# jeremy-rifkin/Markov-Huffman-Coding

Measured on AMD Instinct MI355X. Metric: encode+decode GB/s on 16 GB byte stream, bit-exact round-trip, higher is better.
Workload: dtype u8

## Files before the change

### markov-huffman-coding_amd/csrc/mh_index.hip

```cpp
#include "mh_decode_dev.hpp"

namespace mhk {

__device__ __forceinline__ uint64_t st_pack(uint32_t prev, uint64_t pos) { return (uint64_t(prev) << 56) | pos; }
__device__ __forceinline__ uint32_t st_shift(const IdxParams &p) { return p.order == 2 ? 48u : 56u; }
__device__ __forceinline__ uint64_t st_make(const IdxParams &p, uint32_t ctx, uint64_t pos) { return (uint64_t(ctx) << st_shift(p)) | pos; }
__device__ __forceinline__ uint64_t st_pos(const IdxParams &p, uint64_t s) { return s & ((1ull << st_shift(p)) - 1ull); }
__device__ __forceinline__ uint32_t st_ctx(const IdxParams &p, uint64_t s) { return uint32_t(s >> st_shift(p)); }

__device__ __forceinline__ void idx_fine_entry(const IdxParams &p, uint64_t g, uint32_t prev, uint64_t pos) {
    if (p.fine && p.order != 2 && (g & ((1u << T_SUB_SHIFT) - 1u)) == 0 && (g >> T_SUB_SHIFT) < p.fine_cap)
        p.fine[g >> T_SUB_SHIFT] = (prev << 24) | (uint32_t(pos) & FINE_POS_MASK);
}

template <typename F>
__device__ __forceinline__ uint64_t walk_segment(const IdxParams &p, const DecTables &tabs, const BitSrc &src, uint64_t start,
                                                 uint64_t seg_end, uint32_t &count, bool &bad, F on_symbol, uint32_t *max_used = nullptr) {
    uint64_t pos = st_pos(p, start);
    uint32_t prev = st_ctx(p, start);
    count = 0;
    bad = false;
    if (max_used) *max_used = 0;
    if (pos >= seg_end) return start;
    GranuleCursor bc;
// ... 356 lines not shown
    IdxWs w;
    w.nseg = (nbits + IDX_SEG_BITS_MIN - 1) / IDX_SEG_BITS_MIN;
    w.nblk = (w.nseg + SCAN_BLOCK - 1) / SCAN_BLOCK;
    auto up = [](size_t v) { return (v + 63) & ~size_t(63); };
    w.off_changed = 64;
    w.off_end = up(w.off_changed + IDX_MAX_PASSES * 4);
    w.off_used = up(w.off_end + size_t(w.nseg) * 8);
    w.off_count = up(w.off_used + size_t(w.nseg) * 8);
    w.off_start = up(w.off_count + size_t(w.nseg) * 4);
    w.off_blk = up(w.off_start + size_t(w.nseg) * 8);
    w.total = up(w.off_blk + size_t(w.nblk + 1) * 8);
    w.nseg5 = (nbits + IX_SEG_BITS - 1) / IX_SEG_BITS;
    w.ntile5 = (w.nseg5 + IX_TILE_SEGS - 1) / IX_TILE_SEGS;
    w.ntblk = (w.ntile5 + SCAN_BLOCK - 1) / SCAN_BLOCK;
    w.dirty_cap = w.nseg5 / 4 + 64;
    w.off_e16 = w.off_end;
    w.off_s16 = up(w.off_e16 + size_t(w.nseg5) * 2);
    w.off_c16 = up(w.off_s16 + size_t(w.nseg5) * 2);
    w.off_dirty = up(w.off_c16 + size_t(w.nseg5) * 2 + 64);
    w.off_dirty2 = up(w.off_dirty + size_t(w.dirty_cap) * 4);
    w.off_tcnt = up(w.off_dirty2 + size_t(w.dirty_cap) * 4);
    w.off_tbase = up(w.off_tcnt + size_t(w.ntile5) * 4);
    w.off_tblk = up(w.off_tbase + size_t(w.ntile5) * 8);
    const size_t total5 = up(w.off_tblk + size_t(w.ntblk + 1) * 8);
    if (total5 > w.total) w.total = total5;
    return w;
}
size_t build_index_workspace_bytes(uint64_t nbits) { return idx_ws_layout(nbits).total; }

static void note_index_path(unsigned char *ws, uint32_t path, hipStream_t st) {
    (void)launch_set_word(reinterpret_cast<uint32_t *>(ws + 8), path, st);
}

static bool index_tiles_eligible(const IdxParams &p, const IdxWs &L, uint32_t g, bool allow_long = false) {
    return p.order != 2 && p.tprim && p.tP == 7 && (allow_long || p.max_len <= p.tP + p.tH) && g == 1 && p.nbits >= (1ull << 20) && L.nseg5 < 0xFFFFFFFFull && !getenv("MH_INDEX_NO_TILES");
}
static hipError_t index_tile_states(const IdxParams &p, const IdxWs &L, unsigned char *ws, hipStream_t st, IdxParams &q, bool *ok_out) {
    hipError_t e = hipSuccess;
    q = p;
    q.e16 = reinterpret_cast<uint16_t *>(ws + L.off_e16);
    q.s16 = reinterpret_cast<uint16_t *>(ws + L.off_s16);
    q.c16 = reinterpret_cast<uint16_t *>(ws + L.off_c16);
    q.tile_cnt = reinterpret_cast<uint32_t *>(ws + L.off_tcnt);
    q.tile_base = reinterpret_cast<unsigned long long *>(ws + L.off_tbase);
    q.nseg5 = L.nseg5; q.ntile5 = L.ntile5;
    q.dirty_list = reinterpret_cast<uint32_t *>(ws + L.off_dirty);
    q.dirty_cap = uint32_t(L.dirty_cap < 0xFFFFFFFFull ? L.dirty_cap : 0xFFFFFFFFull);
    const uint64_t dwant = (q.nseg5 + 255) / 256;
    const unsigned dgrid = unsigned(dwant < 2048 ? dwant : 2048);
    bool ok = false;
    uint32_t it = 0;
    q.warm_bits = 256;
    if (const char *wv = getenv("MH_INDEX_WARM_BITS")) { const int v = atoi(wv); if (v >= 16 && v <= int(IX_WARM_BITS_MAX)) q.warm_bits = uint32_t(v); }
    else if (q.ntile5 >= 16384) {
        IdxParams sq = q;
        sq.ntile5 = q.ntile5 / 256 > 4096 ? q.ntile5 / 256 : 4096;
        sq.nseg5 = sq.ntile5 * IX_TILE_SEGS;
        sq.warm_bits = 96;
        sq.iter = it;
        e = launch_index_tile(sq, 0, st);
        if (e != hipSuccess) return e;
        hipLaunchKernelGGL(index_tile_dirty_kernel, dim3(256), dim3(256), 0, st, sq);
        unsigned int dirty = ~0u;
        e = hipMemcpyAsync(&dirty, q.changed + it, 4, hipMemcpyDeviceToHost, st);
        if (e == hipSuccess) e = hipStreamSynchronize(st);
        if (e != hipSuccess) return e;
        ++it;
        if (uint64_t(dirty) * 40u < sq.nseg5) q.warm_bits = 96;
// ... 279 lines not shown
```

### markov-huffman-coding_amd/csrc/mh_tile.hip

```cpp
#include <hip/hip_runtime.h>
#include <stdint.h>

#include <algorithm>
#include <cstdlib>
#include <mutex>
#include <utility>
#include <vector>

#include "mh_kernels.h"
#include "mh_model.hpp"

namespace mhk {

using mh::DEC16_LEAF;

constexpr int T_SUB = 1 << T_SUB_SHIFT;
constexpr int T_TILE = 64 * T_SUB;
constexpr int T_NU = T_SUB / 16;
constexpr int T_LPK = 1024 / T_SUB;
constexpr int T_NG = 64 / T_LPK;
static_assert(T_SUB == 32 || T_SUB == 64, "the output transposition below is written for 32- or 64-symbol sub-chunks");
constexpr int T_THREADS = 1024;
constexpr int T_WAVES = T_THREADS / 64;
constexpr int T_LDS_BYTES = 163840;
// ... 13 lines not shown
template <int O2>
__device__ __forceinline__ uint64_t sub_pos(const TileParams &p, uint64_t j, uint32_t f) {
    return sub_pos_of<O2>(p.index[(j << T_SUB_SHIFT) >> p.chunk_shift], f);
}

__device__ __forceinline__ uint64_t uniform64(uint64_t v) {
    const uint32_t lo = uint32_t(__builtin_amdgcn_readfirstlane(int(uint32_t(v))));
    const uint32_t hi = uint32_t(__builtin_amdgcn_readfirstlane(int(uint32_t(v >> 32))));
    return (uint64_t(hi) << 32) | lo;
}

__device__ __forceinline__ uint64_t stage_first(uint64_t start) { return (start >> 3) & ~uint64_t(15); }

typedef __attribute__((address_space(3))) const uint32_t lds_u32;
typedef uint32_t u32x4 __attribute__((ext_vector_type(4)));
template <typename T>
__device__ __forceinline__ __attribute__((address_space(3))) const T *lds_ptr(uint32_t byte_addr) {
    return reinterpret_cast<__attribute__((address_space(3))) const T *>(byte_addr);
}
template <typename T>
__device__ __forceinline__ __attribute__((address_space(3))) T *lds_wptr(uint32_t byte_addr) {
    return reinterpret_cast<__attribute__((address_space(3))) T *>(byte_addr);
}
__device__ __forceinline__ uint32_t lds_addr_of(const void *generic) {
    return uint32_t(reinterpret_cast<uintptr_t>((__attribute__((address_space(3))) const void *)(generic)));
}

__device__ __forceinline__ unsigned long long tile_stamp() {
    unsigned long long t;
    __builtin_amdgcn_sched_barrier(0);
    asm volatile("s_waitcnt vmcnt(0) lgkmcnt(0)\n\ts_memtime %0\n\ts_waitcnt lgkmcnt(0)" : "=s"(t) :: "memory");
    __builtin_amdgcn_sched_barrier(0);
    return t;
}

__device__ __forceinline__ uint32_t tile_put_byte(uint32_t d, uint32_t e, int j) {
    const uint32_t sel = j == 0 ? 0x03020104u : j == 1 ? 0x03020400u : j == 2 ? 0x03040100u : 0x04020100u;
    return __builtin_amdgcn_perm(e, d, sel);
}

#ifdef MH_EXP_PROBES
#include "mh_tile_probes.hpp"
#else
__host__ __device__ constexpr uint32_t tile_probe_reserve(int) { return 0u; }
#endif

template <int K, int PC, int HC, int OUT, int WIN, int STAMP = 0, int O2 = 0, int G = 0>
__global__ __launch_bounds__(T_THREADS) void decode_tile_kernel(TileParams p) {
    extern __shared__ __attribute__((aligned(16))) unsigned char smem[];
    constexpr uint32_t P = PC;
    const uint32_t PRIM_BYTES = O2 ? ((p.nslots << P) * 4u + 15u) & ~15u : (256u << P) * 2u;
    const uint32_t tid = threadIdx.x, lane = tid & 63u, wave = tid >> 6;
    if (p.d_nbits) {
        p.nbits = *p.d_nbits;
        p.payload_bytes = (p.nbits + 7) >> 3;
    }
    uint16_t *lut = reinterpret_cast<uint16_t *>(smem);
    for (uint32_t i = tid; i < PRIM_BYTES / 16u; i += T_THREADS)
        reinterpret_cast<uint4 *>(lut)[i] = reinterpret_cast<const uint4 *>(p.prim)[i];
    __syncthreads();
    const uint64_t nsub = (p.n + T_SUB - 1) >> T_SUB_SHIFT;
    constexpr uint32_t RESERVE = tile_probe_reserve(G);
    const uint32_t free_bytes = uint32_t(T_LDS_BYTES) - PRIM_BYTES - RESERVE;
    uint32_t maxb;
    {
        uint32_t *s_max = reinterpret_cast<uint32_t *>(smem + PRIM_BYTES + RESERVE);
// ... 321 lines not shown
                        const u32x4 v = *lds_ptr<u32x4>(rb + l * uint32_t(T_SUB) + ((u ^ swz(l)) << 4));
                        reinterpret_cast<uint4 *>(p.out + ((j0 + uint64_t(k) * 64u + uint32_t(g) * uint32_t(T_LPK)) << T_SUB_SHIFT))[lane] = make_uint4(v.x, v.y, v.z, v.w);
                        __builtin_amdgcn_wave_barrier();
                        asm volatile("" ::: "memory");
                    }
                }
            }
            if (STAMP) { const unsigned long long t4 = tile_stamp(); seg[2] += t3 - t2; seg[3] += t4 - t3; }
            land_ahead(seg[1], seg[0]);
        } else {
            if (mc.cls == 1u) {
                if (lane == 0) atomicExch(p.status, MHK_STATUS_CORRUPT);
            } else {
                const uint64_t c0 = (tc * TSYM) >> p.chunk_shift;
                for (uint32_t c = lane; c < chunks_per_tile * K; c += 64) p.redo[1u + atomicAdd(p.redo, 1u)] = uint32_t(c0 + c);
            }
            fetch_ahead();
            land_ahead(seg[1], seg[0]);
        }
    }
    if (STAMP && lane == 0) {
        unsigned long long *dst = reinterpret_cast<unsigned long long *>(p.status) + 1;
        for (int i = 0; i < 4; ++i) atomicAdd(&dst[i], seg[i]);
    }
}

constexpr uint32_t IX_TILE_BYTES = IX_TILE_BITS / 8;
constexpr uint32_t IX_STAGE_LEAD = IX_WARM_BITS_MAX / 8;
constexpr uint32_t IX_STAGE_BYTES = IX_TILE_BYTES + IX_STAGE_LEAD + 32u;
constexpr uint32_t IX_REGION = IX_STAGE_BYTES + 16u;
static_assert(IX_STAGE_LEAD % 16 == 0 && IX_STAGE_BYTES % 16 == 0 && IX_TILE_BYTES % 16 == 0, "16-byte staging loads");
static_assert(IX_TILE_SEGS == 128, "two segments per lane");

template <int MODE, int PC>
__global__ __launch_bounds__(T_THREADS) void index_tile_kernel(IdxParams p) {
    extern __shared__ __attribute__((aligned(16))) unsigned char smem[];
    constexpr uint32_t P = PC, PRIM_BYTES = (256u << P) * 2u;
    constexpr int K = 2;
    const uint32_t tid = threadIdx.x, lane = tid & 63u, wave = tid >> 6;
    for (uint32_t i = tid; i < PRIM_BYTES / 16u; i += T_THREADS)
        reinterpret_cast<uint4 *>(smem)[i] = reinterpret_cast<const uint4 *>(p.tprim)[i];
    __syncthreads();
    constexpr uint32_t NW = (uint32_t(T_LDS_BYTES) - PRIM_BYTES) / IX_REGION < uint32_t(T_WAVES) ? (uint32_t(T_LDS_BYTES) - PRIM_BYTES) / IX_REGION : uint32_t(T_WAVES);
    if (wave >= NW) return;
    if (lds_addr_of(smem) != 0u) {
        if (tid == 0) atomicExch(p.status, MHK_STATUS_CORRUPT);
        return;
    }
    unsigned char *reg = smem + PRIM_BYTES + wave * IX_REGION;
    const uint32_t reg_bit0 = lds_addr_of(reg) * 8u;
    const uint32_t H = p.tH;
    const __amdgpu_buffer_rsrc_t sec_rsrc =
        __builtin_amdgcn_make_buffer_rsrc(const_cast<uint16_t *>(p.tsec), 0, p.tnsec ? int((p.tnsec + 8u) * 2u) : 0, 0x00020000);
    const uint64_t vec_total = (p.payload_bytes + 15u) >> 4;
    const uint64_t cmask = (1ull << p.chunk_shift) - 1ull;

    for (uint64_t t = uint64_t(blockIdx.x) * NW + wave; t < p.ntile5; t += uint64_t(gridDim.x) * NW) {
        const uint64_t sb = t ? t * IX_TILE_BYTES - IX_STAGE_LEAD : 0ull;
        {
            const uint4 *src = reinterpret_cast<const uint4 *>(p.payload + sb);
            const uint64_t left = vec_total - (sb >> 4);
            const uint32_t nvec = left < IX_STAGE_BYTES / 16u ? uint32_t(left) : IX_STAGE_BYTES / 16u;
            for (uint32_t i = lane; i < IX_REGION / 16u; i += 64u) {
                uint4 v = make_uint4(0, 0, 0, 0);
                if (i < nvec) {
                    v = src[i];
                    v.x = __builtin_bswap32(__builtin_bitreverse32(v.x));
                    v.y = __builtin_bswap32(__builtin_bitreverse32(v.y));
                    v.z = __builtin_bswap32(__builtin_bitreverse32(v.z));
                    v.w = __builtin_bswap32(__builtin_bitreverse32(v.w));
                }
                *reinterpret_cast<uint4 *>(reg + i * 16u) = v;
            }
        }
        uint64_t seg[K], base[K];
        uint32_t qb0[K], qe0[K], q[K], ctx[K], k[K], S[K], badv[K], want_e[K], want_c[K], next_entry[K];
        bool active[K], last[K];
#pragma unroll
        for (int j = 0; j < K; ++j) {
            seg[j] = t * IX_TILE_SEGS + uint32_t(j) * 64u + lane;
            const uint64_t b0 = seg[j] * IX_SEG_BITS;
            active[j] = b0 < p.nbits;
            const uint64_t e0 = b0 + IX_SEG_BITS < p.nbits ? b0 + IX_SEG_BITS : p.nbits;
            last[j] = active[j] && e0 == p.nbits;
            qb0[j] = reg_bit0 + uint32_t(b0 - sb * 8u);
            qe0[j] = active[j] ? reg_bit0 + uint32_t(e0 - sb * 8u) : qb0[j];
            k[j] = 0; S[j] = IX_INVALID; badv[j] = DEC16_LEAF; base[j] = 0; want_e[j] = want_c[j] = next_entry[j] = 0;
            if (MODE == 0) {
                const bool exact = seg[j] == 0;
                ctx[j] = exact ? p.prev0 : 0x20u;
                const uint32_t room = qb0[j] - reg_bit0;
                q[j] = exact || !active[j] ? qb0[j] : qb0[j] - (p.warm_bits < room ? p.warm_bits : room);
            } else {
                uint32_t pe = p.prev0 << 8;
                if (active[j] && seg[j]) pe = p.e16[seg[j] - 1];
                ctx[j] = pe >> 8;
                q[j] = active[j] ? qb0[j] + (pe & 255u) : qb0[j];
                want_e[j] = active[j] ? p.e16[seg[j]] : 0u;
                want_c[j] = active[j] ? (p.c16[seg[j]] & IX_C16_COUNT) : 0u;
            }
        }
        if (MODE == 1) {
            uint64_t run = p.tile_base[t];
#pragma unroll
            for (int j = 0; j < K; ++j) {
                uint32_t inc = want_c[j];
#pragma unroll
                for (int d = 1; d < 64; d <<= 1) { const uint32_t o = __shfl_up(inc, d); if (lane >= uint32_t(d)) inc += o; }
                base[j] = run + (inc - want_c[j]);
                next_entry[j] = (0u - uint32_t(base[j])) & ((1u << T_SUB_SHIFT) - 1u);
                run += __shfl(inc, 63);
            }
        }
        uint32_t overflow = 0;
        auto step = [&](auto entered_c) __attribute__((always_inline)) {
            constexpr bool ENTERED = decltype(entered_c)::value;
            if (MODE == 1) {
#pragma unroll
                for (int j = 0; j < K; ++j) {
                    if (q[j] < qe0[j] && k[j] == next_entry[j]) {
                        next_entry[j] += 1u << T_SUB_SHIFT;
                        const uint64_t g = base[j] + k[j];
                        const uint64_t pos = sb * 8u + (q[j] - reg_bit0);
                        if ((g & cmask) == 0) {
                            const uint64_t ci = g >> p.chunk_shift;
                            if (ci < p.index_cap) p.index[ci] = (uint64_t(ctx[j]) << 56) | pos; else overflow = 1;
                        }
                        if (p.fine && (g >> T_SUB_SHIFT) < p.fine_cap) p.fine[g >> T_SUB_SHIFT] = (ctx[j] << 24) | (uint32_t(pos) & FINE_POS_MASK);
                    }
                }
            }
            uint32_t w0[K], w1[K], win[K], e[K], e2[K];
#pragma unroll
            for (int j = 0; j < K; ++j) {
                const lds_u32 *wp = lds_ptr<uint32_t>((q[j] >> 3) & ~3u);
                w0[j] = wp[0];
                w1[j] = wp[1];
            }
            __builtin_amdgcn_sched_barrier(0);
#pragma unroll
            for (int j = 0; j < K; ++j) {
                win[j] = __builtin_amdgcn_alignbit(w1[j], w0[j], q[j]);
                e[j] = *lds_ptr<uint16_t>(((win[j] << 1) & ((2u << P) - 2u)) | (ctx[j] << (P + 1)));
            }
            __builtin_amdgcn_sched_barrier(0);
#pragma unroll
            for (int j = 0; j < K; ++j) {
// ... 11 lines not shown
                    q[j] += __builtin_amdgcn_ubfe(efm, 8, 5);
                    ctx[j] = efm & 255u;
                    k[j] += go ? 1u : 0u;
                } else {
                    const bool in = q[j] >= qb0[j];
                    if (MODE == 0) S[j] = (in && S[j] == IX_INVALID) ? ((ctx[j] << 8) | (q[j] - qb0[j])) : S[j];
                    const uint32_t len = __builtin_amdgcn_ubfe(ef, 8, 5);
                    const bool ok = (ef & DEC16_LEAF) != 0u;
                    badv[j] &= (in && go && !ok) ? 0u : ~0u;
                    ctx[j] = (ok && go) ? (ef & 255u) : ctx[j];
                    q[j] += go ? (ok ? len : 1u) : 0u;
                    k[j] += (in && go) ? 1u : 0u;
                }
            }
        };
        uint32_t it = 0;
        if (MODE == 0) {
#pragma unroll 1
            for (; it < IX_WARM_BITS_MAX + 64u; it += 4u) {
                if (__all(q[0] >= qb0[0] && q[1] >= qb0[1])) break;
#pragma unroll
                for (int sub = 0; sub < 4; ++sub) step(std::false_type{});
            }
#pragma unroll
            for (int j = 0; j < K; ++j)
                S[j] = (q[j] >= qb0[j] && S[j] == IX_INVALID) ? ((ctx[j] << 8) | (q[j] - qb0[j])) : S[j];
        }
#pragma unroll 1
        for (; it < IX_SEG_BITS + IX_WARM_BITS_MAX + 64u; it += 4u) {
            if (!__any(q[0] < qe0[0] || q[1] < qe0[1])) break;
#pragma unroll
            for (int sub = 0; sub < 4; ++sub) step(std::true_type{});
        }
#pragma unroll
        for (int j = 0; j < K; ++j) {
            if (!active[j]) continue;
            const bool done = q[j] >= qe0[j];
            const uint32_t E = (ctx[j] << 8) | (q[j] - qe0[j]);
            if (MODE == 0) {
                if (S[j] == IX_INVALID && done) S[j] = E;
                p.s16[seg[j]] = uint16_t(!(badv[j] & DEC16_LEAF) || !done ? IX_INVALID : S[j]);
                p.e16[seg[j]] = uint16_t(done ? E : IX_INVALID);
                p.c16[seg[j]] = uint16_t(k[j]);
            } else {
                if (!(badv[j] & DEC16_LEAF) || !done || E != want_e[j] || k[j] != want_c[j] || (last[j] && (E & 255u) != 0u)) atomicExch(p.status, MHK_STATUS_CORRUPT);
            }
        }
        if (MODE == 1 && overflow) atomicExch(p.status, MHK_STATUS_CAPACITY);
    }
}

constexpr uint32_t SD_REGION = IX_TILE_BYTES + 48u;
static_assert(SD_REGION % 16 == 0, "16-byte staging stores");
typedef uint32_t u32x4_unaligned __attribute__((ext_vector_type(4), aligned(1)));
typedef uint32_t u32x2_unaligned __attribute__((ext_vector_type(2), aligned(1)));
typedef uint32_t u32_unaligned __attribute__((aligned(1)));
typedef uint16_t u16_unaligned __attribute__((aligned(1)));

constexpr int SD_GROUPS = 5;
constexpr uint32_t SD_ROUND = 16u * SD_GROUPS;
__device__ __forceinline__ void seg_store_run(uint8_t *d, const uint4 (&Qk)[SD_GROUPS], uint32_t m) {
#pragma unroll
    for (int g = 0; g < SD_GROUPS; ++g)
        if (m >= 16u * uint32_t(g + 1)) *reinterpret_cast<u32x4_unaligned *>(d + 16 * g) = u32x4_unaligned{Qk[g].x, Qk[g].y, Qk[g].z, Qk[g].w};
    const uint32_t gt = m >> 4, t = m & 15u;
    if (gt >= uint32_t(SD_GROUPS) || t == 0u) return;
    uint32_t c[SD_GROUPS][4];
#pragma unroll
    for (int g = 0; g < SD_GROUPS; ++g) {
        c[g][0] = Qk[g].x; c[g][1] = Qk[g].y; c[g][2] = Qk[g].z; c[g][3] = Qk[g].w;
#pragma unroll
        for (int i = 0; i < 4; ++i) asm("" : "+v"(c[g][i]));
    }
    uint32_t T[4];
#pragma unroll
    for (int i = 0; i < 4; ++i) {
        T[i] = c[SD_GROUPS - 1][i];
#pragma unroll
        for (int g = SD_GROUPS - 2; g >= 0; --g) T[i] = gt == uint32_t(g) ? c[g][i] : T[i];
    }
    uint8_t *dt = d + 16u * gt;
    if (t & 8u) { *reinterpret_cast<u32x2_unaligned *>(dt) = u32x2_unaligned{T[0], T[1]}; T[0] = T[2]; T[1] = T[3]; dt += 8; }
    if (t & 4u) { *reinterpret_cast<u32_unaligned *>(dt) = T[0]; T[0] = T[1]; dt += 4; }
    if (t & 2u) { *reinterpret_cast<u16_unaligned *>(dt) = uint16_t(T[0]); T[0] >>= 16; dt += 2; }
    if (t & 1u) *dt = uint8_t(T[0]);
}

template <int PC>
__global__ __launch_bounds__(T_THREADS) void segment_decode_kernel(IdxParams p, uint8_t *out, uint64_t out_cap) {
    extern __shared__ __attribute__((aligned(16))) unsigned char smem[];
    constexpr uint32_t P = PC, PRIM_BYTES = (256u << P) * 2u;
    constexpr int K = 2;
    const uint32_t tid = threadIdx.x, lane = tid & 63u, wave = tid >> 6;
    for (uint32_t i = tid; i < PRIM_BYTES / 16u; i += T_THREADS)
        reinterpret_cast<uint4 *>(smem)[i] = reinterpret_cast<const uint4 *>(p.tprim)[i];
    __syncthreads();
    constexpr uint32_t NW = (uint32_t(T_LDS_BYTES) - PRIM_BYTES) / SD_REGION < uint32_t(T_WAVES) ? (uint32_t(T_LDS_BYTES) - PRIM_BYTES) / SD_REGION : uint32_t(T_WAVES);
    if (wave >= NW) return;
    if (lds_addr_of(smem) != 0u) {
        if (tid == 0) atomicExch(p.status, MHK_STATUS_CORRUPT);
        return;
    }
    unsigned char *reg = smem + PRIM_BYTES + wave * SD_REGION;
    const uint32_t reg_bit0 = lds_addr_of(reg) * 8u;
    const uint32_t H = p.tH;
    const __amdgpu_buffer_rsrc_t sec_rsrc =
        __builtin_amdgcn_make_buffer_rsrc(const_cast<uint16_t *>(p.tsec), 0, p.tnsec ? int((p.tnsec + 8u) * 2u) : 0, 0x00020000);
    const uint64_t vec_total = (p.payload_bytes + 15u) >> 4;

    for (uint64_t t = uint64_t(blockIdx.x) * NW + wave; t < p.ntile5; t += uint64_t(gridDim.x) * NW) {
        const uint64_t sb = t * IX_TILE_BYTES;
        {
            const uint4 *src = reinterpret_cast<const uint4 *>(p.payload + sb);
            const uint64_t left = vec_total - (sb >> 4);
            const uint32_t nvec = left < (IX_TILE_BYTES + 32u) / 16u ? uint32_t(left) : (IX_TILE_BYTES + 32u) / 16u;
            for (uint32_t i = lane; i < SD_REGION / 16u; i += 64u) {
                uint4 v = make_uint4(0, 0, 0, 0);
                if (i < nvec) {
                    v = src[i];
                    v.x = __builtin_bswap32(__builtin_bitreverse32(v.x));
                    v.y = __builtin_bswap32(__builtin_bitreverse32(v.y));
                    v.z = __builtin_bswap32(__builtin_bitreverse32(v.z));
                    v.w = __builtin_bswap32(__builtin_bitreverse32(v.w));
                }
                *reinterpret_cast<uint4 *>(reg + i * 16u) = v;
            }
        }
        uint64_t seg[K], base[K];
        uint32_t qe0[K], q[K], ctx[K], k[K], want_e[K], want_c[K], unres[K];
        bool active[K], last[K], skip[K];
#pragma unroll
        for (int j = 0; j < K; ++j) {
            seg[j] = t * IX_TILE_SEGS + uint32_t(j) * 64u + lane;
            const uint64_t b0 = seg[j] * IX_SEG_BITS;
            active[j] = b0 < p.nbits;
            skip[j] = false;
            const uint64_t e0 = b0 + IX_SEG_BITS < p.nbits ? b0 + IX_SEG_BITS : p.nbits;
            last[j] = active[j] && e0 == p.nbits;
            const uint32_t qb0 = reg_bit0 + uint32_t(b0 - sb * 8u);
            qe0[j] = active[j] ? reg_bit0 + uint32_t(e0 - sb * 8u) : qb0;
            uint32_t pe = p.prev0 << 8;
            if (active[j] && seg[j]) pe = p.e16[seg[j] - 1];
            ctx[j] = pe >> 8;
            q[j] = active[j] ? qb0 + (pe & 255u) : qb0;
            want_e[j] = active[j] ? p.e16[seg[j]] : 0u;
            const uint32_t c = active[j] ? p.c16[seg[j]] : 0u;
            want_c[j] = c & IX_C16_COUNT;
            k[j] = 0; unres[j] = DEC16_LEAF;
            if (c & IX_C16_WALK) {
                const uint32_t slot = atomicAdd(&p.changed[IDX_MAX_PASSES - 1], 1u);
                if (slot < p.dirty_cap) p.dirty_list[slot] = uint32_t(seg[j]);
                active[j] = false;
                q[j] = qe0[j];
                skip[j] = true;
            }
        }
        bool fits = true;
        {
            uint64_t run = p.tile_base[t];
#pragma unroll
            for (int j = 0; j < K; ++j) {
                uint32_t inc = want_c[j];
#pragma unroll
                for (int d = 1; d < 64; d <<= 1) { const uint32_t o = __shfl_up(inc, d); if (lane >= uint32_t(d)) inc += o; }
                base[j] = run + (inc - want_c[j]);
                run += __shfl(inc, 63);
                fits = fits && base[j] + want_c[j] <= out_cap;
            }
        }
        if (!__all(fits)) {
            if (lane == 0) atomicExch(p.status, MHK_STATUS_CAPACITY);
            continue;
        }
#pragma unroll 1
        for (uint32_t r = 0; r < (IX_SEG_BITS + SD_ROUND - 1u) / SD_ROUND + 1u; ++r) {
            uint4 Q[K][SD_GROUPS];
#pragma unroll
            for (int j = 0; j < K; ++j)
#pragma unroll
                for (int g = 0; g < SD_GROUPS; ++g) Q[j][g] = make_uint4(0, 0, 0, 0);
            uint32_t ug = 0;
#pragma unroll 1
            for (; ug < uint32_t(SD_GROUPS); ++ug) {
                if (!__any(q[0] < qe0[0] || q[1] < qe0[1])) break;
                uint32_t w4[K][4];
                auto steps8 = [&](auto half_c) __attribute__((always_inline)) {
                    constexpr int J0 = decltype(half_c)::value * 8;
#pragma unroll
                    for (int jj = J0; jj < J0 + 8; ++jj) {
                        uint32_t w0[K], w1[K], win[K], e[K], e2[K];
#pragma unroll
                        for (int j = 0; j < K; ++j) {
                            const lds_u32 *wp = lds_ptr<uint32_t>((q[j] >> 3) & ~3u);
                            w0[j] = wp[0];
                            w1[j] = wp[1];
                        }
                        __builtin_amdgcn_sched_barrier(0);
#pragma unroll
                        for (int j = 0; j < K; ++j) {
                            win[j] = __builtin_amdgcn_alignbit(w1[j], w0[j], q[j]);
                            e[j] = *lds_ptr<uint16_t>(((win[j] << 1) & ((2u << P) - 2u)) | (ctx[j] << (P + 1)));
                        }
                        __builtin_amdgcn_sched_barrier(0);
#pragma unroll
                        for (int j = 0; j < K; ++j) {
                            const uint32_t idx2 = (e[j] << (H + 1)) | ((win[j] >> (P - 1)) & ((2u << H) - 2u));
                            e2[j] = uint32_t(uint16_t(__builtin_amdgcn_raw_buffer_load_b16(sec_rsrc, int(idx2), 0, 0)));
                        }
                        __builtin_amdgcn_sched_barrier(0);
#pragma unroll
                        for (int j = 0; j < K; ++j) {
                            const bool go = q[j] < qe0[j];
                            const uint32_t ef = e[j] > e2[j] ? e[j] : e2[j];
                            const uint32_t efm = go ? ef : (DEC16_LEAF | ctx[j]);
                            unres[j] &= efm;
                            q[j] += __builtin_amdgcn_ubfe(efm, 8, 5);
                            ctx[j] = efm & 255u;
                            k[j] += go ? 1u : 0u;
                            w4[j][jj >> 2] = (jj & 3) == 0 ? ctx[j] : tile_put_byte(w4[j][jj >> 2], efm, jj & 3);
                        }
                    }
                };
                steps8(std::integral_constant<int, 0>{});
#pragma unroll
                for (int j = 0; j < K; ++j) { w4[j][2] = 0; w4[j][3] = 0; }
                if (__any(q[0] < qe0[0] || q[1] < qe0[1])) steps8(std::integral_constant<int, 1>{});
#pragma unroll
                for (int j = 0; j < K; ++j) {
#pragma unroll
                    for (int g = 0; g + 1 < SD_GROUPS; ++g) Q[j][g] = Q[j][g + 1];
                    Q[j][SD_GROUPS - 1] = make_uint4(w4[j][0], w4[j][1], w4[j][2], w4[j][3]);
                }
            }
            if (ug == 0u) break;
            for (uint32_t i = ug; i < uint32_t(SD_GROUPS); ++i) {
#pragma unroll
                for (int j = 0; j < K; ++j)
#pragma unroll
                    for (int g = 0; g + 1 < SD_GROUPS; ++g) Q[j][g] = Q[j][g + 1];
            }
#pragma unroll
            for (int j = 0; j < K; ++j) {
                const uint32_t have = skip[j] ? 0u : (k[j] < want_c[j] ? k[j] : want_c[j]);
                const uint32_t m = have > SD_ROUND * r ? (have - SD_ROUND * r < SD_ROUND ? have - SD_ROUND * r : SD_ROUND) : 0u;
#ifdef MH_EXP_PROBES
                if (p.iter & 1u) continue;
#endif
                if (m) seg_store_run(out + base[j] + SD_ROUND * r, Q[j], m);
            }
        }
#pragma unroll
        for (int j = 0; j < K; ++j) {
            if (!active[j]) continue;
            const bool done = q[j] >= qe0[j];
            const uint32_t E = (ctx[j] << 8) | (q[j] - qe0[j]);
            if (!(unres[j] & DEC16_LEAF) || !done || E != want_e[j] || k[j] != want_c[j] || (last[j] && (E & 255u) != 0u)) atomicExch(p.status, MHK_STATUS_CORRUPT);
        }
    }
}

#ifdef MH_EXP_PROBES
static unsigned tile_grid_cap(unsigned grid) {
    if (const char *g = getenv("MH_TILE_GRID")) {
        const int v = atoi(g);
        if (v > 0 && unsigned(v) < grid) return unsigned(v);
    }
    return grid;
}
#else
static unsigned tile_grid_cap(unsigned grid) { return grid; }
#endif

hipError_t launch_segment_decode(const IdxParams &p, uint8_t *d_out, uint64_t out_cap, hipStream_t st) {
    if (p.tP != 7 || !p.tprim || p.order == 2 || !p.e16 || !p.c16 || !p.tile_base) return hipErrorInvalidValue;
    void (*kern)(IdxParams, uint8_t *, uint64_t) = segment_decode_kernel<7>;
    int dev = 0;
    hipError_t e = hipGetDevice(&dev);
    if (e != hipSuccess) return e;
    {
        static std::mutex mu;
        static std::vector<std::pair<const void *, int>> done;
        std::lock_guard<std::mutex> lock(mu);
        const std::pair<const void *, int> key(reinterpret_cast<const void *>(kern), dev);
        if (std::find(done.begin(), done.end(), key) == done.end()) {
            e = hipFuncSetAttribute(key.first, hipFuncAttributeMaxDynamicSharedMemorySize, T_LDS_BYTES);
            if (e != hipSuccess) return e;
            done.push_back(key);
        }
    }
    int cus = 0;
    if (hipDeviceGetAttribute(&cus, hipDeviceAttributeMultiprocessorCount, dev) != hipSuccess || cus <= 0) cus = 256;
    const uint64_t want = (p.ntile5 + T_WAVES - 1) / T_WAVES;
    const unsigned grid = tile_grid_cap(unsigned(want < 1 ? 1 : (want > uint64_t(cus) ? uint64_t(cus) : want)));
#ifdef MH_EXP_PROBES
    if (const char *pr = getenv("MH_SEG_PROBE")) { IdxParams pp = p; pp.iter = uint32_t(atoi(pr)); hipLaunchKernelGGL(kern, dim3(grid), dim3(T_THREADS), T_LDS_BYTES, st, pp, d_out, out_cap); return hipGetLastError(); }
#endif
    hipLaunchKernelGGL(kern, dim3(grid), dim3(T_THREADS), T_LDS_BYTES, st, p, d_out, out_cap);
    return hipGetLastError();
}

hipError_t launch_index_tile(const IdxParams &p, int mode, hipStream_t st) {
    if (p.tP != 7 || !p.tprim || p.order == 2) return hipErrorInvalidValue;
    if (mode == 0 && (p.warm_bits == 0 || p.warm_bits > IX_WARM_BITS_MAX)) return hipErrorInvalidValue;
    void (*kern)(IdxParams) = mode == 0 ? index_tile_kernel<0, 7> : index_tile_kernel<1, 7>;
    int dev = 0;
    hipError_t e = hipGetDevice(&dev);
    if (e != hipSuccess) return e;
    {
        static std::mutex mu;
        static std::vector<std::pair<const void *, int>> done;
        std::lock_guard<std::mutex> lock(mu);
        const std::pair<const void *, int> key(reinterpret_cast<const void *>(kern), dev);
        if (std::find(done.begin(), done.end(), key) == done.end()) {
            e = hipFuncSetAttribute(key.first, hipFuncAttributeMaxDynamicSharedMemorySize, T_LDS_BYTES);
            if (e != hipSuccess) return e;
            done.push_back(key);
        }
    }
    int cus = 0;
    if (hipDeviceGetAttribute(&cus, hipDeviceAttributeMultiprocessorCount, dev) != hipSuccess || cus <= 0) cus = 256;
    const uint64_t want = (p.ntile5 + T_WAVES - 1) / T_WAVES;
    const unsigned grid = tile_grid_cap(unsigned(want < 1 ? 1 : (want > uint64_t(cus) ? uint64_t(cus) : want)));
    hipLaunchKernelGGL(kern, dim3(grid), dim3(T_THREADS), T_LDS_BYTES, st, p);
    return hipGetLastError();
}


size_t decode_tile_workspace_extra() { return 64; }


template <int K, int O2 = 0>
static hipError_t launch_tile_with(void (*kern)(TileParams), TileParams p, const DecParams &legacy, void *d_ws, hipStream_t st) {
    int dev = 0;
    hipError_t e = hipGetDevice(&dev);
    if (e != hipSuccess) return e;
    {
        static std::mutex mu;
// ... 46 lines not shown
#ifdef MH_EXP_PROBES
    if (const char *pr = getenv("MH_TILE_PROBE")) { p.probe = uint32_t(atoi(pr)); if (p.probe & 1) p.nsec = 0; }
    const char *e = getenv("MH_TILE_K");
    const int k = e ? atoi(e) : 2;
    const char *eo = getenv("MH_TILE_OUT");
    const int o = eo ? atoi(eo) : 2;
    if (o == 1) return k == 1 ? launch_tile_k<1, 1>(p, legacy, d_ws, st) : launch_tile_k<2, 1>(p, legacy, d_ws, st);
    if (const char *es = getenv("MH_TILE_STAMP")) {
        if (atoi(es)) {
            void (*ks)(TileParams) = decode_tile_kernel<2, 7, 0, 2, 0, 1>;
            if (p.P != 7) return hipErrorInvalidValue;
            return launch_tile_with<2>(ks, p, legacy, d_ws, st);
        }
    }
    if (const char *eg = getenv("MH_TILE_G")) {
        const int g = atoi(eg), w = getenv("MH_TILE_WIN") ? atoi(getenv("MH_TILE_WIN")) : 0;
        if (g && p.P != 7) return hipErrorInvalidValue;
        void (*kg)(TileParams) = nullptr;
#define MH_G_CASE(GV) case GV: kg = k == 1 ? (w ? decode_tile_kernel<1, 7, 0, 2, 1, 0, 0, GV> : decode_tile_kernel<1, 7, 0, 2, 0, 0, 0, GV>) \
                                           : (w ? decode_tile_kernel<2, 7, 0, 2, 1, 0, 0, GV> : decode_tile_kernel<2, 7, 0, 2, 0, 0, 0, GV>); break;
        switch (g) { MH_G_CASE(1) MH_G_CASE(2) MH_G_CASE(3) MH_G_CASE(4) MH_G_CASE(5) MH_G_CASE(6) MH_G_CASE(7) default: break; }
#undef MH_G_CASE
        if (kg) return k == 1 ? launch_tile_with<1>(kg, p, legacy, d_ws, st) : launch_tile_with<2>(kg, p, legacy, d_ws, st);
    }
    const char *ew = getenv("MH_TILE_WIN");
    if (ew && atoi(ew) == 1) return k == 4 ? launch_tile_k<4, 2, 1>(p, legacy, d_ws, st) : k == 3 ? launch_tile_k<3, 2, 1>(p, legacy, d_ws, st) : launch_tile_k<2, 2, 1>(p, legacy, d_ws, st);
    return k == 1 ? launch_tile_k<1, 2>(p, legacy, d_ws, st) : k == 4 ? launch_tile_k<4, 2>(p, legacy, d_ws, st) : k == 3 ? launch_tile_k<3, 2>(p, legacy, d_ws, st) : launch_tile_k<2, 2>(p, legacy, d_ws, st);
#else
    return launch_tile_k<2, 2>(p, legacy, d_ws, st);
#endif
}

}
```

Baseline: 564.6.

## Software-pipeline payload and state fetches in index and segment-decode tile kernels

Restructures the persistent tile loops of index_tile_kernel and segment_decode_kernel so that the payload bytes and per-segment entry/count states for the next tile are loaded into registers while the current tile is still being processed. The data is written to LDS only after the current tile finishes. This is meant to hide global-memory latency that was previously exposed at the start of each tile. The cost is extra vector registers for the prefetch buffers, which may reduce occupancy or cause spills. It also adds probe-only timestamp instrumentation and environment knobs that choose where the prefetch is placed.

Measured after the change: 564.1. Within noise of the previous version (-0.1%).

```diff
diff --git a/markov-huffman-coding_amd/csrc/mh_index.hip b/markov-huffman-coding_amd/csrc/mh_index.hip
--- a/markov-huffman-coding_amd/csrc/mh_index.hip
+++ b/markov-huffman-coding_amd/csrc/mh_index.hip
@@ -412,8 +412,19 @@
     (void)launch_set_word(reinterpret_cast<uint32_t *>(ws + 8), path, st);
 }
 
+#ifdef MH_EXP_PROBES
+static uint64_t index_tiles_min_bits() {
+    if (const char *s = getenv("MH_INDEX_MIN_BITS")) {
+        const long long v = atoll(s);
+        if (v > 0 && v < (1ll << 20)) return uint64_t(v);
+    }
+    return 1ull << 20;
+}
+#else
+static uint64_t index_tiles_min_bits() { return 1ull << 20; }
+#endif
 static bool index_tiles_eligible(const IdxParams &p, const IdxWs &L, uint32_t g, bool allow_long = false) {
-    return p.order != 2 && p.tprim && p.tP == 7 && (allow_long || p.max_len <= p.tP + p.tH) && g == 1 && p.nbits >= (1ull << 20) && L.nseg5 < 0xFFFFFFFFull && !getenv("MH_INDEX_NO_TILES");
+    return p.order != 2 && p.tprim && p.tP == 7 && (allow_long || p.max_len <= p.tP + p.tH) && g == 1 && p.nbits >= index_tiles_min_bits() && L.nseg5 < 0xFFFFFFFFull && !getenv("MH_INDEX_NO_TILES");
 }
 static hipError_t index_tile_states(const IdxParams &p, const IdxWs &L, unsigned char *ws, hipStream_t st, IdxParams &q, bool *ok_out) {
     hipError_t e = hipSuccess;
diff --git a/markov-huffman-coding_amd/csrc/mh_tile.hip b/markov-huffman-coding_amd/csrc/mh_tile.hip
--- a/markov-huffman-coding_amd/csrc/mh_tile.hip
+++ b/markov-huffman-coding_amd/csrc/mh_tile.hip
@@ -69,6 +69,26 @@
     asm volatile("s_waitcnt vmcnt(0) lgkmcnt(0)\n\ts_memtime %0\n\ts_waitcnt lgkmcnt(0)" : "=s"(t) :: "memory");
     __builtin_amdgcn_sched_barrier(0);
     return t;
+}
+
+#ifdef MH_EXP_PROBES
+__device__ unsigned long long ix_stamp_acc[3][4];
+#endif
+template <bool DRAIN>
+__device__ __forceinline__ unsigned long long ix_stamp() {
+    if (DRAIN) return tile_stamp();
+    unsigned long long t;
+    __builtin_amdgcn_sched_barrier(0);
+    asm volatile("s_waitcnt lgkmcnt(0)\n\ts_memtime %0\n\ts_waitcnt lgkmcnt(0)" : "=s"(t) :: "memory");
+    __builtin_amdgcn_sched_barrier(0);
+    return t;
+}
+template <int ROW>
+__device__ __forceinline__ void ix_stamp_flush(const unsigned long long (&ph)[4], uint32_t lane) {
+#ifdef MH_EXP_PROBES
+    if (lane == 0)
+        for (int i = 0; i < 4; ++i) atomicAdd(&ix_stamp_acc[ROW][i], ph[i]);
+#endif
 }
 
 __device__ __forceinline__ uint32_t tile_put_byte(uint32_t d, uint32_t e, int j) {
@@ -456,7 +476,66 @@
 static_assert(IX_STAGE_LEAD % 16 == 0 && IX_STAGE_BYTES % 16 == 0 && IX_TILE_BYTES % 16 == 0, "16-byte staging loads");
 static_assert(IX_TILE_SEGS == 128, "two segments per lane");
 
-template <int MODE, int PC>
+constexpr int IX_NPF = 6;
+template <int K>
+struct IxStates { uint32_t pe[K], we[K], wc[K]; uint64_t tb; };
+
+__device__ __forceinline__ uint32_t ix_nvec(uint64_t sb, uint64_t vec_total, uint32_t max_vec) {
+    const uint64_t left = vec_total - (sb >> 4);
+    return left < max_vec ? uint32_t(left) : max_vec;
+}
+__device__ __forceinline__ uint32_t ix_opaque_zero() {
+    uint32_t z = 0u;
+    asm volatile("" : "+v"(z));
+    return z;
+}
+template <bool KEEP>
+__device__ __forceinline__ void ix_fetch_payload(const uint8_t *payload, uint64_t sb, uint32_t nvec, uint32_t lane, uint4 (&V)[IX_NPF]) {
+    uint64_t sb_far = sb + 4096u;
+    asm volatile("" : "+s"(sb_far));
+    const uint4 *src = reinterpret_cast<const uint4 *>(payload + sb), *src_far = reinterpret_cast<const uint4 *>(payload + sb_far);
+#pragma unroll
+    for (int i = 0; i < IX_NPF; ++i) {
+        if (!KEEP) { const uint32_t z = ix_opaque_zero(); V[i] = make_uint4(z, z, z, z); }
+        if (lane + 64u * uint32_t(i) < nvec) V[i] = i < 4 ? src[lane + 64u * uint32_t(i)] : src_far[lane + 64u * uint32_t(i - 4)];
+    }
+}
+template <uint32_t REGION_VECS>
+__device__ __forceinline__ void ix_land_payload(uint32_t reg_addr, uint32_t nvec, uint32_t lane, const uint4 (&V)[IX_NPF]) {
+    static_assert(REGION_VECS <= 64u * IX_NPF, "the region is what one batch fetches");
+#pragma unroll
+    for (int i = 0; i < IX_NPF; ++i) {
+        const uint32_t v = lane + 64u * uint32_t(i);
+        const bool have = v < nvec;
+        if (64u * uint32_t(i + 1) <= REGION_VECS || v < REGION_VECS)
+            *lds_wptr<u32x4>(reg_addr + v * 16u) = u32x4{have ? __builtin_bswap32(__builtin_bitreverse32(V[i].x)) : 0u, have ? __builtin_bswap32(__builtin_bitreverse32(V[i].y)) : 0u,
+                                                         have ? __builtin_bswap32(__builtin_bitreverse32(V[i].z)) : 0u, have ? __builtin_bswap32(__builtin_bitreverse32(V[i].w)) : 0u};
+    }
+}
+template <int K, bool KEEP>
+__device__ __forceinline__ void ix_fetch_states(const IdxParams &p, uint64_t t, uint32_t lane, IxStates<K> &s) {
+#pragma unroll
+    for (int j = 0; j < K; ++j) {
+        const uint64_t seg = t * IX_TILE_SEGS + uint32_t(j) * 64u + lane;
+        const bool active = seg * IX_SEG_BITS < p.nbits;
+        if (!KEEP) s.pe[j] = s.we[j] = s.wc[j] = ix_opaque_zero();
+        uint64_t in_front = seg - 1;
+        asm volatile("" : "+v"(in_front));
+        if (active && seg) s.pe[j] = p.e16[in_front];
+        if (active) { s.we[j] = p.e16[seg]; s.wc[j] = p.c16[seg]; }
+    }
+    s.tb = p.tile_base[t];
+}
+template <int K>
+__device__ __forceinline__ void ix_states_of(const IdxParams &p, uint64_t t, uint32_t lane, const IxStates<K> &s, int j, uint32_t &pe, uint32_t &we, uint32_t &wc) {
+    const uint64_t seg = t * IX_TILE_SEGS + uint32_t(j) * 64u + lane;
+    const bool active = seg * IX_SEG_BITS < p.nbits;
+    pe = active && seg ? s.pe[j] : p.prev0 << 8;
+    we = active ? s.we[j] : 0u;
+    wc = active ? s.wc[j] : 0u;
+}
+
+template <int MODE, int PC, int STAMP = 0, int PL = 0>
 __global__ __launch_bounds__(T_THREADS) void index_tile_kernel(IdxParams p) {
     extern __shared__ __attribute__((aligned(16))) unsigned char smem[];
     constexpr uint32_t P = PC, PRIM_BYTES = (256u << P) * 2u;
@@ -478,25 +557,33 @@
         __builtin_amdgcn_make_buffer_rsrc(const_cast<uint16_t *>(p.tsec), 0, p.tnsec ? int((p.tnsec + 8u) * 2u) : 0, 0x00020000);
     const uint64_t vec_total = (p.payload_bytes + 15u) >> 4;
     const uint64_t cmask = (1ull << p.chunk_shift) - 1ull;
-
-    for (uint64_t t = uint64_t(blockIdx.x) * NW + wave; t < p.ntile5; t += uint64_t(gridDim.x) * NW) {
-        const uint64_t sb = t ? t * IX_TILE_BYTES - IX_STAGE_LEAD : 0ull;
-        {
-            const uint4 *src = reinterpret_cast<const uint4 *>(p.payload + sb);
-            const uint64_t left = vec_total - (sb >> 4);
-            const uint32_t nvec = left < IX_STAGE_BYTES / 16u ? uint32_t(left) : IX_STAGE_BYTES / 16u;
-            for (uint32_t i = lane; i < IX_REGION / 16u; i += 64u) {
-                uint4 v = make_uint4(0, 0, 0, 0);
-                if (i < nvec) {
-                    v = src[i];
-                    v.x = __builtin_bswap32(__builtin_bitreverse32(v.x));
-                    v.y = __builtin_bswap32(__builtin_bitreverse32(v.y));
-                    v.z = __builtin_bswap32(__builtin_bitreverse32(v.z));
-                    v.w = __builtin_bswap32(__builtin_bitreverse32(v.w));
-                }
-                *reinterpret_cast<uint4 *>(reg + i * 16u) = v;
-            }
-        }
+    unsigned long long ph[4] = {0, 0, 0, 0}, s0 = 0, s1 = 0, s2 = 0, s3 = 0;
+
+    const uint64_t stride = uint64_t(gridDim.x) * NW;
+    uint64_t t = uint64_t(blockIdx.x) * NW + uint32_t(__builtin_amdgcn_readfirstlane(int(wave)));
+    if (t >= p.ntile5) return;
+    const uint32_t reg_addr = lds_addr_of(reg);
+    auto first_byte = [](uint64_t tile) -> uint64_t { return tile ? tile * IX_TILE_BYTES - IX_STAGE_LEAD : 0ull; };
+    uint4 V[IX_NPF];
+    IxStates<K> nx;
+#pragma unroll
+    for (int i = 0; i < IX_NPF; ++i) V[i] = make_uint4(0, 0, 0, 0);
+#pragma unroll
+    for (int j = 0; j < K; ++j) nx.pe[j] = nx.we[j] = nx.wc[j] = 0u;
+    nx.tb = 0;
+    auto nvec_of = [&](uint64_t tile) -> uint32_t { return ix_nvec(first_byte(tile), vec_total, IX_STAGE_BYTES / 16u); };
+    auto fetch = [&](uint64_t tile) __attribute__((always_inline)) {
+        __builtin_amdgcn_sched_barrier(0);
+        ix_fetch_payload<true>(p.payload, first_byte(tile), nvec_of(tile), lane, V);
+        if (MODE == 1) ix_fetch_states<K, true>(p, tile, lane, nx);
+        __builtin_amdgcn_sched_barrier(0);
+    };
+    if (STAMP) s0 = ix_stamp<false>();
+    fetch(t);
+    ix_land_payload<IX_REGION / 16u>(reg_addr, nvec_of(t), lane, V);
+    for (;;) {
+        const uint64_t sb = first_byte(t), tn = t + stride;
+        if (STAMP) s1 = ix_stamp<false>();
         uint64_t seg[K], base[K];
         uint32_t qb0[K], qe0[K], q[K], ctx[K], k[K], S[K], badv[K], want_e[K], want_c[K], next_entry[K];
         bool active[K], last[K];
@@ -516,16 +603,16 @@
                 const uint32_t room = qb0[j] - reg_bit0;
                 q[j] = exact || !active[j] ? qb0[j] : qb0[j] - (p.warm_bits < room ? p.warm_bits : room);
             } else {
-                uint32_t pe = p.prev0 << 8;
-                if (active[j] && seg[j]) pe = p.e16[seg[j] - 1];
+                uint32_t pe, we, wc;
+                ix_states_of<K>(p, t, lane, nx, j, pe, we, wc);
                 ctx[j] = pe >> 8;
                 q[j] = active[j] ? qb0[j] + (pe & 255u) : qb0[j];
-                want_e[j] = active[j] ? p.e16[seg[j]] : 0u;
-                want_c[j] = active[j] ? (p.c16[seg[j]] & IX_C16_COUNT) : 0u;
+                want_e[j] = we;
+                want_c[j] = wc & IX_C16_COUNT;
             }
         }
         if (MODE == 1) {
-            uint64_t run = p.tile_base[t];
+            uint64_t run = nx.tb;
 #pragma unroll
             for (int j = 0; j < K; ++j) {
                 uint32_t inc = want_c[j];
@@ -537,6 +624,8 @@
             }
         }
         uint32_t overflow = 0;
+        if (STAMP) s2 = ix_stamp<false>();
+        if (PL == 0 && tn < p.ntile5) fetch(tn);
         auto step = [&](auto entered_c) __attribute__((always_inline)) {
             constexpr bool ENTERED = decltype(entered_c)::value;
             if (MODE == 1) {
@@ -614,6 +703,8 @@
 #pragma unroll
             for (int sub = 0; sub < 4; ++sub) step(std::true_type{});
         }
+        if (STAMP) s3 = ix_stamp<false>();
+        if (PL == 1 && tn < p.ntile5) fetch(tn);
 #pragma unroll
         for (int j = 0; j < K; ++j) {
             if (!active[j]) continue;
@@ -629,7 +720,12 @@
             }
         }
         if (MODE == 1 && overflow) atomicExch(p.status, MHK_STATUS_CAPACITY);
-    }
+        if (STAMP) { const unsigned long long s4 = ix_stamp<false>(); ph[0] += s1 - s0; ph[1] += s2 - s1; ph[2] += s3 - s2; ph[3] += s4 - s3; s0 = s4; }
+        if (tn >= p.ntile5) break;
+        ix_land_payload<IX_REGION / 16u>(reg_addr, nvec_of(tn), lane, V);
+        t = tn;
+    }
+    if (STAMP) ix_stamp_flush<MODE>(ph, lane);
 }
 
 constexpr uint32_t SD_REGION = IX_TILE_BYTES + 48u;
@@ -668,7 +764,7 @@
     if (t & 1u) *dt = uint8_t(T[0]);
 }
 
-template <int PC>
+template <int PC, int STAMP = 0>
 __global__ __launch_bounds__(T_THREADS) void segment_decode_kernel(IdxParams p, uint8_t *out, uint64_t out_cap) {
     extern __shared__ __attribute__((aligned(16))) unsigned char smem[];
     constexpr uint32_t P = PC, PRIM_BYTES = (256u << P) * 2u;
@@ -689,25 +785,28 @@
     const __amdgpu_buffer_rsrc_t sec_rsrc =
         __builtin_amdgcn_make_buffer_rsrc(const_cast<uint16_t *>(p.tsec), 0, p.tnsec ? int((p.tnsec + 8u) * 2u) : 0, 0x00020000);
     const uint64_t vec_total = (p.payload_bytes + 15u) >> 4;
-
-    for (uint64_t t = uint64_t(blockIdx.x) * NW + wave; t < p.ntile5; t += uint64_t(gridDim.x) * NW) {
-        const uint64_t sb = t * IX_TILE_BYTES;
-        {
-            const uint4 *src = reinterpret_cast<const uint4 *>(p.payload + sb);
-            const uint64_t left = vec_total - (sb >> 4);
-            const uint32_t nvec = left < (IX_TILE_BYTES + 32u) / 16u ? uint32_t(left) : (IX_TILE_BYTES + 32u) / 16u;
-            for (uint32_t i = lane; i < SD_REGION / 16u; i += 64u) {
-                uint4 v = make_uint4(0, 0, 0, 0);
-                if (i < nvec) {
-                    v = src[i];
-                    v.x = __builtin_bswap32(__builtin_bitreverse32(v.x));
-                    v.y = __builtin_bswap32(__builtin_bitreverse32(v.y));
-                    v.z = __builtin_bswap32(__builtin_bitreverse32(v.z));
-                    v.w = __builtin_bswap32(__builtin_bitreverse32(v.w));
-                }
-                *reinterpret_cast<uint4 *>(reg + i * 16u) = v;
-            }
-        }
+    unsigned long long ph[4] = {0, 0, 0, 0}, s0 = 0, s1 = 0, s2 = 0, s3 = 0;
+
+    const uint64_t stride = uint64_t(gridDim.x) * NW;
+    uint64_t t = uint64_t(blockIdx.x) * NW + uint32_t(__builtin_amdgcn_readfirstlane(int(wave)));
+    if (t >= p.ntile5) return;
+    const uint32_t reg_addr = lds_addr_of(reg);
+    uint4 V[IX_NPF];
+    IxStates<K> nx;
+    auto nvec_of = [&](uint64_t tile) -> uint32_t { return ix_nvec(tile * IX_TILE_BYTES, vec_total, (IX_TILE_BYTES + 32u) / 16u); };
+    auto fetch = [&](uint64_t tile) __attribute__((always_inline)) {
+        __builtin_amdgcn_sched_barrier(0);
+        ix_fetch_payload<false>(p.payload, tile * IX_TILE_BYTES, nvec_of(tile), lane, V);
+        ix_fetch_states<K, false>(p, tile, lane, nx);
+        __builtin_amdgcn_sched_barrier(0);
+    };
+    if (STAMP) s0 = ix_stamp<false>();
+    fetch(t);
+    ix_land_payload<SD_REGION / 16u>(reg_addr, nvec_of(t), lane, V);
+    for (;;) {
+        const uint64_t sb = t * IX_TILE_BYTES, tn = t + stride;
+        const bool more = tn < p.ntile5;
+        if (STAMP) s1 = ix_stamp<false>();
         uint64_t seg[K], base[K];
         uint32_t qe0[K], q[K], ctx[K], k[K], want_e[K], want_c[K], unres[K];
         bool active[K], last[K], skip[K];
@@ -721,12 +820,10 @@
             last[j] = active[j] && e0 == p.nbits;
             const uint32_t qb0 = reg_bit0 + uint32_t(b0 - sb * 8u);
             qe0[j] = active[j] ? reg_bit0 + uint32_t(e0 - sb * 8u) : qb0;
-            uint32_t pe = p.prev0 << 8;
-            if (active[j] && seg[j]) pe = p.e16[seg[j] - 1];
+            uint32_t pe, c;
+            ix_states_of<K>(p, t, lane, nx, j, pe, want_e[j], c);
             ctx[j] = pe >> 8;
             q[j] = active[j] ? qb0 + (pe & 255u) : qb0;
-            want_e[j] = active[j] ? p.e16[seg[j]] : 0u;
-            const uint32_t c = active[j] ? p.c16[seg[j]] : 0u;
             want_c[j] = c & IX_C16_COUNT;
             k[j] = 0; unres[j] = DEC16_LEAF;
             if (c & IX_C16_WALK) {
@@ -739,7 +836,7 @@
         }
         bool fits = true;
         {
-            uint64_t run = p.tile_base[t];
+            uint64_t run = nx.tb;
 #pragma unroll
             for (int j = 0; j < K; ++j) {
                 uint32_t inc = want_c[j];
@@ -750,12 +847,14 @@
                 fits = fits && base[j] + want_c[j] <= out_cap;
             }
         }
-        if (!__all(fits)) {
+        const bool fits_all = __all(fits);
+        if (STAMP) { s2 = ix_stamp<false>(); ph[0] += s1 - s0; ph[1] += s2 - s1; }
+        if (!fits_all) {
             if (lane == 0) atomicExch(p.status, MHK_STATUS_CAPACITY);
-            continue;
-        }
+        } else {
 #pragma unroll 1
         for (uint32_t r = 0; r < (IX_SEG_BITS + SD_ROUND - 1u) / SD_ROUND + 1u; ++r) {
+            if (STAMP) s2 = ix_stamp<false>();
             uint4 Q[K][SD_GROUPS];
 #pragma unroll
             for (int j = 0; j < K; ++j)
@@ -814,6 +913,7 @@
                     Q[j][SD_GROUPS - 1] = make_uint4(w4[j][0], w4[j][1], w4[j][2], w4[j][3]);
                 }
             }
+            if (STAMP) { s3 = ix_stamp<false>(); ph[2] += s3 - s2; }
             if (ug == 0u) break;
             for (uint32_t i = ug; i < uint32_t(SD_GROUPS); ++i) {
 #pragma unroll
@@ -830,7 +930,9 @@
 #endif
                 if (m) seg_store_run(out + base[j] + SD_ROUND * r, Q[j], m);
             }
-        }
+            if (STAMP) ph[3] += ix_stamp<false>() - s3;
+        }
+        if (STAMP) s3 = ix_stamp<false>();
 #pragma unroll
         for (int j = 0; j < K; ++j) {
             if (!active[j]) continue;
@@ -838,7 +940,15 @@
             const uint32_t E = (ctx[j] << 8) | (q[j] - qe0[j]);
             if (!(unres[j] & DEC16_LEAF) || !done || E != want_e[j] || k[j] != want_c[j] || (last[j] && (E & 255u) != 0u)) atomicExch(p.status, MHK_STATUS_CORRUPT);
         }
-    }
+        if (STAMP) ph[3] += ix_stamp<false>() - s3;
+        }
+        if (more) fetch(tn);
+        if (STAMP) s0 = ix_stamp<false>();
+        if (!more) break;
+        ix_land_payload<SD_REGION / 16u>(reg_addr, nvec_of(tn), lane, V);
+        t = tn;
+    }
+    if (STAMP) ix_stamp_flush<2>(ph, lane);
 }
 
 #ifdef MH_EXP_PROBES
@@ -849,6 +959,14 @@
     }
     return grid;
 }
+static bool ix_stamp_wanted() {
+    const char *s = getenv("MH_IX_STAMP");
+    return s && atoi(s) != 0;
+}
+static int ix_place(int shipped) {
+    const char *s = getenv("MH_IX_PLACE");
+    return s ? (atoi(s) != 0 ? 1 : 0) : shipped;
+}
 #else
 static unsigned tile_grid_cap(unsigned grid) { return grid; }
 #endif
@@ -856,6 +974,9 @@
 hipError_t launch_segment_decode(const IdxParams &p, uint8_t *d_out, uint64_t out_cap, hipStream_t st) {
     if (p.tP != 7 || !p.tprim || p.order == 2 || !p.e16 || !p.c16 || !p.tile_base) return hipErrorInvalidValue;
     void (*kern)(IdxParams, uint8_t *, uint64_t) = segment_decode_kernel<7>;
+#ifdef MH_EXP_PROBES
+    if (ix_stamp_wanted()) kern = segment_decode_kernel<7, 1>;
+#endif
     int dev = 0;
     hipError_t e = hipGetDevice(&dev);
     if (e != hipSuccess) return e;
@@ -885,6 +1006,11 @@
     if (p.tP != 7 || !p.tprim || p.order == 2) return hipErrorInvalidValue;
     if (mode == 0 && (p.warm_bits == 0 || p.warm_bits > IX_WARM_BITS_MAX)) return hipErrorInvalidValue;
     void (*kern)(IdxParams) = mode == 0 ? index_tile_kernel<0, 7> : index_tile_kernel<1, 7>;
+#ifdef MH_EXP_PROBES
+    if (ix_place(0) == 1) kern = ix_stamp_wanted() ? (mode == 0 ? index_tile_kernel<0, 7, 1, 1> : index_tile_kernel<1, 7, 1, 1>)
+                                                   : (mode == 0 ? index_tile_kernel<0, 7, 0, 1> : index_tile_kernel<1, 7, 0, 1>);
+    else if (ix_stamp_wanted()) kern = mode == 0 ? index_tile_kernel<0, 7, 1, 0> : index_tile_kernel<1, 7, 1, 0>;
+#endif
     int dev = 0;
     hipError_t e = hipGetDevice(&dev);
     if (e != hipSuccess) return e;
@@ -997,3 +1123,15 @@
 }
 
 }
+
+#ifdef MH_EXP_PROBES
+extern "C" __attribute__((visibility("default"))) int mh_diag_index_stamps(unsigned long long *out12, int reset) {
+    hipError_t e = hipDeviceSynchronize();
+    if (e == hipSuccess && out12) e = hipMemcpyFromSymbol(out12, HIP_SYMBOL(mhk::ix_stamp_acc), sizeof(mhk::ix_stamp_acc));
+    if (e == hipSuccess && reset) {
+        const unsigned long long zero[12] = {0};
+        e = hipMemcpyToSymbol(HIP_SYMBOL(mhk::ix_stamp_acc), zero, sizeof(zero));
+    }
+    return e == hipSuccess ? 0 : -1;
+}
+#endif
```
